# YihongSun/Dynamo-Depth

Measured on AMD Instinct MI355X. Metric: training images/sec (192x640 triplets), higher is better.
Workload: dtype f32

## Files before the change

### dynamo-depth_amd/hipops/abi.py

```python
import ctypes as C

DD_MAX_SCALES = 4
DD_NUM_SRC = 2
DD_ABI_VERSION = 2
DD_MODE_RIGID, DD_MODE_FLOW, DD_MODE_FLOW_MASK = 0, 1, 2
DD_PARTIAL_STRIDE = 40
DD_SUMS_STRIDE = 8

_fp = C.c_void_p


class DDPhotoScale(C.Structure):
    _fields_ = [
        ("shift", C.c_int), ("h", C.c_int), ("w", C.c_int),
        ("w_photo", C.c_float), ("w_cons", C.c_float),
        ("disp", _fp),
        ("flow", _fp * DD_NUM_SRC),
        ("mask", _fp * DD_NUM_SRC),
        ("noise", _fp),
        ("g_disp", _fp),
        ("g_flow", _fp * DD_NUM_SRC),
        ("g_mask", _fp * DD_NUM_SRC),
        ("out_color", _fp * DD_NUM_SRC),
        ("out_sample", _fp * DD_NUM_SRC),
# ... 123 lines not shown
        "dd_dwconv3x3_nhwc": (i, [v, v, i, i, i, i, i, v, v]),
        "dd_dwconv3x3_nhwc_bwd_data": (i, [v, v, i, i, i, i, i, v, v]),
        "dd_dwconv3x3_nhwc_bwd_weight": (i, [v, v, i, i, i, i, i, v, v, z, v]),
        "dd_dwconv3x3_workspace_bytes": (z, [i, i, i]),
        "dd_conv3x3_cout1_bwd_data": (i, [v, v, i, i, i, i, i, v, v]),
        "dd_prepare_frames": (i, [v, v, v, i, i, i, i, v, v, v, v]),
        "dd_prepare_frames_workspace_bytes": (z, [i, i]),
        "dd_pyramid_down2": (i, [v, i, i, i, v, v]),
        "dd_pack_rgb": (i, [v, i, i, i, v, v]),
        "dd_depth_metrics": (i, [v, i, i, i, v, v, i, v, C.POINTER(C.c_double), f, f, v, v, v, z, v]),
        "dd_depth_metrics_workspace_bytes": (z, [i, i]),
        "dd_depth_metrics_masked": (i, [v, i, i, i, v, v, i, v, C.POINTER(C.c_double), f, f, v, i, i, v, v, v, v, z, v]),
        "dd_depth_metrics_masked_workspace_bytes": (z, [i, i]),
        "dd_depth_metrics_accumulate": (i, [v, v, i, v, v, v]),
        "dd_odom_snippet_count": (i, [i, i]),
        "dd_odom_snippets": (i, [v, v, i, i, v, v, v]),
        "dd_motion_pr": (i, [v, i, i, i, v, v, i, i, v, i, i, v, v]),
        "dd_fill_contours": (i, [v, i, v, i, i, i, i, v, v]),
        "dd_vis_frame": (i, [v, v, v, v, v, v, v, v, f, f, i, i, C.POINTER(C.c_int), i, i, i, v, f, f, f, f, i, i, v, v, v, v]),
        "dd_vis_flow_tiles": (i, [v, v, C.POINTER(C.c_int), i, i, i, i, i, i, f, i, v, v]),
        "dd_bn_act_fwd": (i, [v, v, C.c_longlong, i, v, v, f, f, v, v, v, v, i, v, v, z, v]),
        "dd_bn_act_bwd": (i, [v, v, v, C.c_longlong, i, v, v, v, v, i, v, v, v, v, v, z, v]),
        "dd_bn_workspace_bytes": (z, [i]),
        "dd_bn_act_fwd_t": (i, [v, v, C.c_longlong, i, v, v, f, f, v, v, v, v, i, v, i, v, z, v]),
        "dd_bn_act_bwd_t": (i, [v, v, v, C.c_longlong, i, v, v, v, v, i, v, v, v, v, i, v, z, v]),
        "dd_channel_sum_nhwc_t": (i, [v, C.c_longlong, i, v, i, v, v]),
        "dd_reflect_pad1_nhwc_t": (i, [v, i, i, i, i, v, i, v]),
        "dd_reflect_pad1_nhwc_bwd_t": (i, [v, i, i, i, i, v, i, v]),
        "dd_up_cat_pad_t": (i, [v, v, i, i, i, i, i, i, i, v, i, v]),
        "dd_up_cat_pad_bwd_t": (i, [v, v, i, i, i, i, i, i, i, v, v, i, v]),
        "dd_layer_norm_fwd": (i, [v, C.c_longlong, i, v, v, f, v, v, v, v]),
        "dd_layer_norm_bwd": (i, [v, v, v, v, v, C.c_longlong, i, v, v, v, z, v]),
        "dd_layer_norm_workspace_bytes": (z, [i]),
        "dd_layer_scale_bwd": (i, [v, v, v, i, i, i, v, v, v, z, v]),
        "dd_layer_scale_workspace_bytes": (z, [i, i]),
        "dd_layer_norm_fwd_t": (i, [v, C.c_longlong, i, v, v, f, v, v, v, i, v]),
        "dd_layer_norm_bwd_t": (i, [v, v, v, v, v, C.c_longlong, i, v, v, v, z, i, v]),
        "dd_layer_scale_bwd_t": (i, [v, v, v, i, i, i, v, v, v, z, i, v]),
        "dd_layer_scale_fwd_t": (i, [v, v, v, i, i, i, v, i, v]),
        "dd_dwconv3x3_nhwc_t": (i, [v, v, i, i, i, i, i, v, i, v]),
        "dd_dwconv3x3_nhwc_bwd_data_t": (i, [v, v, i, i, i, i, i, v, i, v]),
        "dd_dwconv3x3_nhwc_bwd_weight_t": (i, [v, v, i, i, i, i, i, v, v, z, i, v]),
        "dd_redu_supported": (i, [i, i]),
        "dd_redu_workspace_bytes": (z, [C.c_longlong, i, i]),
        "dd_redu_fwd": (i, [v, v, v, v, C.c_longlong, i, i, v, v]),
        "dd_redu_bwd_data": (i, [v, v, C.c_longlong, i, i, v, v, v]),
        "dd_redu_bwd_weight": (i, [v, v, v, C.c_longlong, i, i, v, v, v, z, v]),
        "dd_conv_head_supported": (i, [i]),
        "dd_conv_head_workspace_bytes": (z, [i, i, i, i]),
        "dd_conv_head_fwd": (i, [v, v, C.c_longlong, C.c_longlong, C.c_longlong, v, i, i, i, i, v, v]),
        "dd_conv_head_bwd_weight": (i, [v, v, i, i, i, i, v, v, v, z, v]),
        "dd_conv_small_supported": (i, [i, i, i]),
        "dd_conv_small_workspace_bytes": (z, [i, i, i]),
        "dd_conv_small_fwd": (i, [v, v, C.c_longlong, C.c_longlong, C.c_longlong, C.c_longlong, v, i, i, i, i, i, i, v, v, z, v]),
        "dd_conv_small_bwd_data": (i, [v, v, C.c_longlong, C.c_longlong, C.c_longlong, C.c_longlong, i, i, i, i, i, i, v, v, z, v]),
        "dd_conv_small_bwd_weight": (i, [v, v, i, i, i, i, i, i, v, v, v, z, v]),
        "dd_conv3x3_mfma_supported": (i, [i, i]),
        "dd_conv3x3_mfma_pack_bytes": (z, [i, i]),
        "dd_conv3x3_mfma_pack": (i, [v, C.c_longlong, C.c_longlong, C.c_longlong, C.c_longlong, i, i, v, v, v]),
        "dd_conv3x3_mfma_pack_many_job_words": (i, []),
        "dd_conv3x3_mfma_pack_many_blocks": (i, [i, i, i, i]),
        "dd_conv3x3_mfma_pack_many": (i, [v, v, i, v]),
        "dd_conv3x3_mfma": (i, [v, v, v, i, i, i, i, i, i, v, v]),
        "dd_conv3x3_mfma_n": (i, [v, v, v, i, i, i, i, i, i, i, v, v]),
        "dd_conv3x3_mfma_flat_supported": (i, [i, i, i, i, i]),
        "dd_conv3x3_mfma_flat_workspace_bytes": (z, [i, i, i, i, i]),
        "dd_conv3x3_mfma_flat": (i, [v, v, v, i, i, i, i, i, v, v, z, v]),
        "dd_conv3x3_mfma_flat_n": (i, [v, v, v, i, i, i, i, i, i, v, v, z, v]),
        "dd_conv3x3_mfma_wgrad_workspace_bytes": (z, [i, i, i, i, i]),
        "dd_conv3x3_mfma_bwd_weight": (i, [v, v, i, i, i, i, i, i, v, v, z, v]),
        "dd_conv3x3_mfma_bwd_weight_n": (i, [v, v, i, i, i, i, i, i, i, v, v, z, v]),
        "dd_conv3x3_half_supported": (i, [i, i]),
        "dd_conv3x3_half_pack_bytes": (z, [i, i]),
        "dd_conv3x3_half_pack": (i, [v, C.c_longlong, C.c_longlong, C.c_longlong, C.c_longlong, i, i, i, v, v, v]),
        "dd_conv3x3_half": (i, [v, v, v, i, i, i, i, i, i, i, v, v]),
        "dd_conv3x3_half_wgrad_workspace_bytes": (z, [i, i, i, i, i]),
        "dd_conv3x3_half_bwd_weight": (i, [v, v, i, i, i, i, i, i, i, v, v, z, v]),
        "dd_pw_gemm_pack_bytes": (z, [i, i]),
        "dd_mlp_pack": (i, [v, C.c_longlong, C.c_longlong, v, C.c_longlong, C.c_longlong, i, i, v, v, v, v, v, v]),
        "dd_mlp_fwd_supported": (i, [i]),
        "dd_mlp_fwd": (i, [v, v, v, v, v, i, i, v, v]),
        "dd_pw_gemm": (i, [v, v, v, i, i, i, i, v, v]),
        "dd_gelu_pair": (i, [v, v, v, z, v]),
        "dd_adam_chunk": (i, []),
        "dd_adam_multi": (i, [v, i, v, i, v, C.c_double, C.c_double, C.c_double, C.c_double, C.c_double, v, v, v]),
        "dd_error_string": (C.c_char_p, [i]),
        "dd_abi_version": (i, []),
    }
    found = []
    for name, (res, args) in sig.items():
        try:
            fn = getattr(lib, name)
        except AttributeError:
            continue
        fn.restype = res
        fn.argtypes = args
        found.append(name)
    return found


EXPORTED = (
    "dd_photo_loss", "dd_photo_workspace_bytes", "dd_photo_timing", "dd_photo_timing_read", "dd_photo_loss_part", "dd_smooth_loss", "dd_smooth_workspace_bytes",
    "dd_ground_loss", "dd_ground_workspace_bytes", "dd_ground_plane", "dd_ground_candidates", "dd_ground_select",
    "dd_assemble_losses", "dd_reg_losses_finish", "dd_fused_loss", "dd_fused_loss_part", "dd_fused_loss_supported", "dd_reg_workspace_bytes", "dd_backproject", "dd_backproject_bwd", "dd_project3d", "dd_project3d_bwd", "dd_project3d_workspace_bytes",
    "dd_ssim", "dd_ssim_bwd", "dd_disp_to_depth", "dd_pose_matrix", "dd_pose_matrix_bwd",
    "dd_channel_sum_nhwc", "dd_channel_sum_workspace_bytes", "dd_reflect_pad1_nhwc", "dd_reflect_pad1_nhwc_bwd",
    "dd_dwconv3x3_nhwc", "dd_dwconv3x3_nhwc_bwd_data", "dd_dwconv3x3_nhwc_bwd_weight", "dd_dwconv3x3_workspace_bytes", "dd_conv3x3_cout1_bwd_data",
    "dd_prepare_frames", "dd_prepare_frames_workspace_bytes", "dd_pyramid_down2", "dd_pack_rgb", "dd_depth_metrics", "dd_depth_metrics_workspace_bytes", "dd_depth_metrics_masked", "dd_depth_metrics_masked_workspace_bytes", "dd_depth_metrics_accumulate", "dd_odom_snippet_count", "dd_odom_snippets", "dd_motion_pr", "dd_fill_contours", "dd_vis_frame", "dd_vis_flow_tiles", "dd_bn_act_fwd", "dd_bn_act_bwd", "dd_bn_workspace_bytes",
    "dd_bn_act_fwd_t", "dd_bn_act_bwd_t", "dd_channel_sum_nhwc_t", "dd_reflect_pad1_nhwc_t", "dd_reflect_pad1_nhwc_bwd_t", "dd_up_cat_pad_t", "dd_up_cat_pad_bwd_t",
    "dd_layer_norm_fwd", "dd_layer_norm_bwd", "dd_layer_norm_workspace_bytes", "dd_layer_scale_bwd", "dd_layer_scale_workspace_bytes",
    "dd_jpeg_workspace_bytes", "dd_jpeg_decode", "dd_resize_workspace_bytes", "dd_resize_bicubic", "dd_layer_norm_fwd_t", "dd_layer_norm_bwd_t", "dd_layer_scale_bwd_t", "dd_layer_scale_fwd_t", "dd_dwconv3x3_nhwc_t", "dd_dwconv3x3_nhwc_bwd_data_t",
    "dd_dwconv3x3_nhwc_bwd_weight_t", "dd_adam_chunk", "dd_adam_multi", "dd_conv_small_supported", "dd_conv_small_workspace_bytes",
    "dd_conv_small_fwd", "dd_conv_small_bwd_data", "dd_conv_small_bwd_weight", "dd_conv_head_supported", "dd_conv_head_workspace_bytes", "dd_conv_head_fwd",
    "dd_conv_head_bwd_weight", "dd_redu_supported", "dd_redu_workspace_bytes", "dd_redu_fwd", "dd_redu_bwd_data", "dd_redu_bwd_weight",
    "dd_conv3x3_mfma_supported", "dd_conv3x3_mfma_pack_bytes", "dd_conv3x3_mfma_pack", "dd_conv3x3_mfma_pack_many_job_words",
    "dd_conv3x3_mfma_pack_many_blocks", "dd_conv3x3_mfma_pack_many", "dd_conv3x3_mfma", "dd_conv3x3_mfma_n",
    "dd_conv3x3_mfma_flat_supported", "dd_conv3x3_mfma_flat_workspace_bytes", "dd_conv3x3_mfma_flat", "dd_conv3x3_mfma_flat_n",
    "dd_conv3x3_mfma_wgrad_workspace_bytes", "dd_conv3x3_mfma_bwd_weight", "dd_conv3x3_mfma_bwd_weight_n",
    "dd_conv3x3_half_supported", "dd_conv3x3_half_pack_bytes", "dd_conv3x3_half_pack", "dd_conv3x3_half",
    "dd_conv3x3_half_wgrad_workspace_bytes", "dd_conv3x3_half_bwd_weight",
    "dd_pw_gemm_pack_bytes", "dd_mlp_pack", "dd_pw_gemm", "dd_gelu_pair", "dd_mlp_fwd_supported", "dd_mlp_fwd",
    "dd_error_string", "dd_abi_version",
)


def fill_photo_args(*, B, H, W, mode, automask, want_grad, min_depth, max_depth, ssim_weight, eps, disp_thr,
                    target, source, K, inv_K, T, ts, g_T, sums, workspace, scales, source_packed=None):
    a = DDPhotoArgs()
    a.abi_version = DD_ABI_VERSION
    a.B, a.H, a.W = B, H, W
    a.num_scales = len(scales)
    a.mode, a.automask, a.want_grad = mode, int(bool(automask)), int(bool(want_grad))
    a.min_depth, a.max_depth, a.ssim_weight, a.eps, a.disp_thr = min_depth, max_depth, ssim_weight, eps, disp_thr
    a.target = ptr(target)
    a.K, a.inv_K = ptr(K), ptr(inv_K)
    a.sums, a.workspace = ptr(sums), ptr(workspace)
    for f in range(DD_NUM_SRC):
        a.source[f] = ptr(source[f])
        a.source_packed[f] = ptr(source_packed[f]) if source_packed is not None else None
        a.T[f] = ptr(T[f])
        a.ts[f] = ptr(ts[f]) if ts is not None else None
        a.g_T[f] = ptr(g_T[f]) if g_T is not None else None
    for s, d in enumerate(scales):
        sc = a.scale[s]
        sc.shift, sc.h, sc.w = d["shift"], d["h"], d["w"]
        sc.w_photo, sc.w_cons = d.get("w_photo", 0.0), d.get("w_cons", 0.0)
        for name in ("disp", "noise", "g_disp", "out_depth", "out_idsel"):
            setattr(sc, name, ptr(d.get(name)))
        for name in ("flow", "mask", "g_flow", "g_mask", "out_color", "out_sample", "out_resid", "out_delta"):
            pair = d.get(name) or (None, None)
            arr = getattr(sc, name)
            for f in range(DD_NUM_SRC):
                arr[f] = ptr(pair[f])
    return a
```

### dynamo-depth_amd/hipops/functions.py

```python
import os

import torch

from . import lib as L
from .pack_many import PackSet, _ACTIVE_PACK_SETS, _pack_many_on, pack_many_launches, pack_weights_once_per_forward


def _dev(t, name="tensor"):
    if not t.is_cuda:
        raise L.DynamoHipError("%s must live on the GPU: the Dynamo-Depth loss path has no CPU implementation "
                               "(libdynamo_hip.so is the only backend)" % name)
    if t.dtype != torch.float32:
        raise L.DynamoHipError("%s must be float32, got %s" % (name, t.dtype))
    return t.contiguous()


DTYPE_CODE = {torch.float32: 0, torch.float16: 1, torch.bfloat16: 2}


def _p(t):
    return None if t is None else t.data_ptr()


def _ws(nbytes, device):
    return torch.empty(max(int(nbytes) // 4, 1), dtype=torch.float32, device=device)


_WS_BYTES = {}


def _ws_bytes(name, *dims):
    key = (name,) + dims
    n = _WS_BYTES.get(key)
    if n is None:
        n = _WS_BYTES[key] = int(getattr(L.load(), name)(*dims))
    return n


def _nhwc_empty(B, Cc, H, W, device, *, dtype=torch.float32):
    return torch.empty((B, H, W, Cc), dtype=dtype, device=device).permute(0, 3, 1, 2)


def _channel_sum(g, rows, cout, code, stream):
    gb = torch.empty(cout, dtype=torch.float32, device=g.device)
    ws = _ws(_ws_bytes("dd_channel_sum_workspace_bytes", cout), g.device)
    L.check(L.load().dd_channel_sum_nhwc_t(_p(g), rows, cout, _p(gb), code, _p(ws), stream), "dd_channel_sum_nhwc_t")
    return gb


def _wgrad_1x1(go, x, w, B, H, W):
    cout, cin = w.shape
    _, gw, _ = torch.ops.aten.convolution_backward(go.view(B, H, W, cout).permute(0, 3, 1, 2), x.view(B, H, W, cin).permute(0, 3, 1, 2),
                                                   w.view(cout, cin, 1, 1), None, [1, 1], [0, 0], [1, 1], False, [0, 0], 1, [False, True, False])
    return gw.reshape(cout, cin)


def _wgrad_3x3_library(g, x, w_like, pad):
    return torch.ops.aten.convolution_backward(g, x, w_like, None, (1, 1), (pad, pad), (1, 1), False, [0, 0], 1, (False, True, False))[1]


def _conv3x3_s1(x, weight, stride, padding, dilation, groups, allowed):
    return (tuple(weight.shape[2:]) == (3, 3) and groups == 1 and tuple(stride) == (1, 1) and tuple(dilation) == (1, 1)
            and tuple(padding) in allowed and x.shape[1] == weight.shape[1])


def _below_tile_pixels(B, Ho, Wo, env_name):
    return Ho < 8 or Wo < 32 or B * Ho * Wo < int(os.environ.get(env_name, "20000"))


class BackprojectFn(torch.autograd.Function):

    @staticmethod
    def forward(ctx, depth, inv_K):
        depth, inv_K = _dev(depth, "depth"), _dev(inv_K, "inv_K")
        B, _, h, w = depth.shape
        pts = torch.empty(B, 4, h * w, dtype=torch.float32, device=depth.device)
        L.check(L.load().dd_backproject(_p(depth), _p(inv_K), B, h, w, _p(pts), L.current_stream()), "dd_backproject")
        ctx.save_for_backward(inv_K)
        ctx.shape = (B, h, w)
        return pts

    @staticmethod
    def backward(ctx, g):
        (inv_K,) = ctx.saved_tensors
        B, h, w = ctx.shape
        g = _dev(g, "grad")
        gd = torch.empty(B, 1, h, w, dtype=torch.float32, device=g.device)
        L.check(L.load().dd_backproject_bwd(_p(g), _p(inv_K), B, h, w, _p(gd), L.current_stream()), "dd_backproject_bwd")
        return gd, None


class Project3DFn(torch.autograd.Function):

    @staticmethod
    def forward(ctx, points, K, T, h, w, eps):
        points, K = _dev(points, "points"), _dev(K, "K")
        T = None if T is None else _dev(T, "T")
        B = points.shape[0]
        pix = torch.empty(B, h, w, 2, dtype=torch.float32, device=points.device)
        ego = torch.empty(B, 3, h * w, dtype=torch.float32, device=points.device)
        L.check(L.load().dd_project3d(_p(points), _p(K), _p(T), B, h, w, eps, _p(pix), _p(ego), L.current_stream()), "dd_project3d")
        ctx.save_for_backward(points, K, T if T is not None else torch.empty(0, device=points.device))
        ctx.has_T = T is not None
        ctx.dims = (B, h, w, eps)
        return pix, ego

    @staticmethod
    def backward(ctx, g_pix, g_ego):
        points, K, T = ctx.saved_tensors
        B, h, w, eps = ctx.dims
        T = T if ctx.has_T else None
        g_pix = None if g_pix is None else _dev(g_pix, "g_pix")
        g_ego = None if g_ego is None else _dev(g_ego, "g_ego")
        lib = L.load()
        g_points = torch.empty_like(points)
        g_T = torch.empty(B, 4, 4, dtype=torch.float32, device=points.device) if T is not None else None
        ws = _ws(lib.dd_project3d_workspace_bytes(B, h, w), points.device)
        L.check(lib.dd_project3d_bwd(_p(points), _p(K), _p(T), _p(g_pix), _p(g_ego), B, h, w, eps, _p(g_points), _p(g_T), _p(ws),
                                     L.current_stream()), "dd_project3d_bwd")
        return g_points, None, g_T, None, None, None


class SSIMFn(torch.autograd.Function):

    @staticmethod
    def forward(ctx, x, y):
        x, y = _dev(x, "x"), _dev(y, "y")
        B, Cc, H, W = x.shape
        out = torch.empty_like(x)
        L.check(L.load().dd_ssim(_p(x), _p(y), B, Cc, H, W, _p(out), L.current_stream()), "dd_ssim")
        ctx.save_for_backward(x, y)
        return out

    @staticmethod
    def backward(ctx, g):
        x, y = ctx.saved_tensors
        B, Cc, H, W = x.shape
# ... 562 lines not shown
    if os.environ.get("DD_STOCK_DECODER_GLUE", "0") == "1":
        return False
    if not (x.is_cuda and x.dtype in DTYPE_CODE and x.dim() == 4 and x.shape[1] % 4 == 0 and x.shape[1] >= 4 and _nhwc(x)
            and x.shape[2] >= 2 and x.shape[3] >= 2 and (mode != 2 or (x.shape[2] >= 4 and x.shape[3] >= 4))):
        return False
    if skip is not None:
        H, W = (x.shape[2], x.shape[3]) if mode == 2 else (2 * x.shape[2], 2 * x.shape[3])
        if not (skip.dtype == x.dtype and skip.is_cuda and skip.shape[0] == x.shape[0] and skip.shape[1] % 4 == 0 and tuple(skip.shape[2:]) == (H, W)
                and _nhwc(skip)):
            return False
    return True


def up_cat_pad(x, skip=None, mode="bilinear", elu=True):
    code = {"nearest": 0, "bilinear": 1, None: 2}[mode]
    if up_cat_pad_ok(x, skip, code):
        return UpCatPadFn.apply(x, skip, code, bool(elu))
    F = torch.nn.functional
    y = F.elu(x) if elu else x
    if mode is not None:
        y = F.interpolate(y, scale_factor=2, mode=mode)
    if skip is not None:
        y = torch.cat((y, skip), 1)
    return reflect_pad1(y)


class DepthwiseConv3x3NHWCFn(torch.autograd.Function):

    @staticmethod
    def forward(ctx, x, weight, dilation):
        B, Cc, H, W = x.shape
        w = weight.contiguous()
        out = torch.empty((B, Cc, H, W), dtype=x.dtype, device=x.device, memory_format=torch.channels_last)
        L.check(L.load().dd_dwconv3x3_nhwc_t(_p(x), _p(w), B, H, W, Cc, dilation, _p(out), DTYPE_CODE[x.dtype], L.current_stream()), "dd_dwconv3x3_nhwc_t")
        ctx.save_for_backward(x, w)
        ctx.dilation = dilation
        return out

    @staticmethod
    def backward(ctx, g):
        x, w = ctx.saved_tensors
        B, Cc, H, W = x.shape
        g = g.to(x.dtype).contiguous(memory_format=torch.channels_last)
        lib, gx, gw = L.load(), None, None
        code = DTYPE_CODE[x.dtype]
        if ctx.needs_input_grad[0]:
            gx = torch.empty((B, Cc, H, W), dtype=x.dtype, device=g.device, memory_format=torch.channels_last)
            L.check(lib.dd_dwconv3x3_nhwc_bwd_data_t(_p(g), _p(w), B, H, W, Cc, ctx.dilation, _p(gx), code, L.current_stream()), "dd_dwconv3x3_nhwc_bwd_data_t")
        if ctx.needs_input_grad[1]:
            gw = torch.empty_like(w)
            nbytes = _ws_bytes("dd_dwconv3x3_workspace_bytes", B, H, Cc)
            ws = _ws(nbytes, g.device)
            L.check(lib.dd_dwconv3x3_nhwc_bwd_weight_t(_p(g), _p(x), B, H, W, Cc, ctx.dilation, _p(gw), _p(ws), nbytes, code, L.current_stream()),
                    "dd_dwconv3x3_nhwc_bwd_weight_t")
        return gx, gw, None


def depthwise_conv3x3(x, weight, dilation):
    Cc = x.shape[1]
    if (x.is_cuda and x.dtype in DTYPE_CODE and weight.dtype == torch.float32 and x.dim() == 4 and Cc % 4 == 0 and Cc <= 512
            and x.is_contiguous(memory_format=torch.channels_last) and not x.is_contiguous()):
        return DepthwiseConv3x3NHWCFn.apply(x, weight, dilation)
    return torch.nn.functional.conv2d(x, weight, None, 1, dilation, dilation, Cc)


class PointwiseLinearFn(torch.autograd.Function):

    @staticmethod
    def forward(ctx, x, weight, bias):
        B, H, W, cin = x.shape
        ctx.save_for_backward(x, weight)
        with torch.autocast("cuda", enabled=False):
            return torch.addmm(bias, x.reshape(-1, cin), weight.t()).view(B, H, W, weight.shape[0])

    @staticmethod
    def backward(ctx, g):
        x, weight = ctx.saved_tensors
        B, H, W, cin = x.shape
        cout = weight.shape[0]
        g = g.to(x.dtype).contiguous()
        gx = gw = gb = None
        if ctx.needs_input_grad[0]:
            gx = torch.mm(g.view(-1, cout), weight).view(B, H, W, cin)
        if ctx.needs_input_grad[1]:
            gw = _wgrad_1x1(g, x, weight, B, H, W)
        if ctx.needs_input_grad[2]:
            gb = _channel_sum(g, B * H * W, cout, DTYPE_CODE[g.dtype], L.current_stream()).to(weight.dtype)
        return gx, gw, gb


def pointwise_linear(x, layer):
    if (x.is_cuda and x.dtype in DTYPE_CODE and layer.weight.dtype == torch.float32 and layer.bias is not None and x.dim() == 4
            and x.is_contiguous() and torch.is_grad_enabled() and layer.out_features <= 4096):
        if torch.is_autocast_enabled():
            dt = torch.get_autocast_dtype("cuda")
            return PointwiseLinearFn.apply(x.to(dt), layer.weight.to(dt), layer.bias.to(dt))
        if x.dtype == torch.float32:
            return PointwiseLinearFn.apply(x, layer.weight, layer.bias)
    return layer(x.reshape(-1, x.shape[-1])).view(*x.shape[:-1], layer.out_features)


_MLP_CALLS = [0]


def mlp_calls():
    return _MLP_CALLS[0]


def mlp_ok(y, block):
    if os.environ.get("DD_MLP", "0") != "1" or os.environ.get("DD_STOCK_MLP", "0") == "1" or torch.is_autocast_enabled():
        return False
    l1, l2 = block.pwconv1, block.pwconv2
    if y.dim() != 4 or y.shape[0] * y.shape[1] * y.shape[2] < int(os.environ.get("DD_MLP_MIN_ROWS", "16384")):
        return False
    return bool(y.is_cuda and y.dtype == torch.float32 and y.dim() == 4 and y.is_contiguous() and l1.weight.dtype == torch.float32
                and l1.bias is not None and l2.bias is not None and l1.in_features % 32 == 0 and l1.out_features % 32 == 0
                and l2.in_features == l1.out_features and l2.out_features == l1.in_features and y.shape[-1] == l1.in_features
                and isinstance(block.act, torch.nn.GELU) and getattr(block.act, "approximate", "none") == "none")


def _mlp_param_grads(needs, g, gpre, y, post, w1, w2, B, H, W, stream):
    M, code = B * H * W, DTYPE_CODE[torch.float32]
    gw1 = _wgrad_1x1(gpre, y, w1, B, H, W) if needs[1] else None
    gb1 = _channel_sum(gpre, M, w1.shape[0], code, stream) if needs[2] else None
    gw2 = _wgrad_1x1(g, post, w2, B, H, W) if needs[3] else None
    gb2 = _channel_sum(g, M, w2.shape[0], code, stream) if needs[4] else None
    return gw1, gb1, gw2, gb2


class MlpFn(torch.autograd.Function):

    @staticmethod
    def forward(ctx, y, w1, b1, w2, b2):
        lib = L.load()
        B, H, W, Cc = y.shape
        hid, M = w1.shape[0], B * H * W
        need = any(ctx.needs_input_grad)
        nb1, nb2 = _ws_bytes("dd_pw_gemm_pack_bytes", hid, Cc), _ws_bytes("dd_pw_gemm_pack_bytes", Cc, hid)
        packs = torch.empty(((nb1 + nb2) * (2 if need else 1)) // 4, dtype=torch.float32, device=y.device)
        p0 = packs.data_ptr()
        stream = L.current_stream()
        L.check(lib.dd_mlp_pack(_p(w1), w1.stride(0), w1.stride(1), _p(w2), w2.stride(0), w2.stride(1), Cc, hid, p0, p0 + nb1,
                                p0 + nb1 + nb2 if need else None, p0 + 2 * nb1 + nb2 if need else None, None, stream), "dd_mlp_pack")
        pre = torch.empty((M, hid), dtype=torch.float32, device=y.device)
        L.check(lib.dd_pw_gemm(_p(y), p0, _p(b1), M, Cc, hid, 0, _p(pre), stream), "dd_pw_gemm (pwconv1)")
        out = torch.empty((B, H, W, Cc), dtype=torch.float32, device=y.device)
        L.check(lib.dd_pw_gemm(_p(pre), p0 + nb1, _p(b2), M, hid, Cc, 1, _p(out), stream), "dd_pw_gemm (GELU, pwconv2)")
        _MLP_CALLS[0] += 1
        if need:
            ctx.save_for_backward(y, pre, w1, w2, packs)
        return out

    @staticmethod
    def backward(ctx, g):
        y, pre, w1, w2, packs = ctx.saved_tensors
        lib = L.load()
        B, H, W, Cc = y.shape
        hid, M = w1.shape[0], B * H * W
        nb1, nb2 = _ws_bytes("dd_pw_gemm_pack_bytes", hid, Cc), _ws_bytes("dd_pw_gemm_pack_bytes", Cc, hid)
        p0 = packs.data_ptr()
        stream = L.current_stream()
        g = g.to(torch.float32).contiguous()
        gpre = torch.empty((M, hid), dtype=torch.float32, device=g.device)
        L.check(lib.dd_pw_gemm(_p(g), p0 + nb1 + nb2, None, M, Cc, hid, 0, _p(gpre), stream), "dd_pw_gemm (g . w2)")
        post = torch.empty((M, hid), dtype=torch.float32, device=g.device)
        L.check(lib.dd_gelu_pair(_p(pre), _p(gpre), _p(post), M * hid, stream), "dd_gelu_pair")
        gy = None
        if ctx.needs_input_grad[0]:
            gy = torch.empty((B, H, W, Cc), dtype=torch.float32, device=g.device)
            L.check(lib.dd_pw_gemm(_p(gpre), p0 + 2 * nb1 + nb2, None, M, hid, Cc, 0, _p(gy), stream), "dd_pw_gemm (g_pre . w1)")
        return (gy,) + _mlp_param_grads(ctx.needs_input_grad, g, gpre, y, post, w1, w2, B, H, W, stream)


def mlp(y, block):
    return MlpFn.apply(y, block.pwconv1.weight, block.pwconv1.bias, block.pwconv2.weight, block.pwconv2.bias)


_MLP_FUSED_CALLS = [0]


def mlp_fused_calls():
    return _MLP_FUSED_CALLS[0]


def _mlp_block_ok(y, block):
    l1, l2 = block.pwconv1, block.pwconv2
    if not (y.is_cuda and y.dtype == torch.float32 and y.dim() == 4 and y.is_contiguous() and l1.weight.dtype == torch.float32):
        return False
    if y.shape[0] * y.shape[1] * y.shape[2] < int(os.environ.get("DD_MLP_FUSED_MIN_ROWS", "16384")):
        return False
    return bool(l1.bias is not None and l2.bias is not None and l1.out_features == 6 * l1.in_features and l2.in_features == l1.out_features
                and l2.out_features == l1.in_features and y.shape[-1] == l1.in_features and isinstance(block.act, torch.nn.GELU)
                and getattr(block.act, "approximate", "none") == "none" and L.load().dd_mlp_fwd_supported(l1.in_features))


def _mlp_fwd_launch(y, w1, b1, w2, b2):
    lib = L.load()
    B, H, W, Cc = y.shape
    hid, M = w1.shape[0], B * H * W
    nb1, nb2 = _ws_bytes("dd_pw_gemm_pack_bytes", hid, Cc), _ws_bytes("dd_pw_gemm_pack_bytes", Cc, hid)
    packs = torch.empty((nb1 + nb2) // 4, dtype=torch.float32, device=y.device)
    p0, stream = packs.data_ptr(), L.current_stream()
    L.check(lib.dd_mlp_pack(_p(w1), w1.stride(0), w1.stride(1), _p(w2), w2.stride(0), w2.stride(1), Cc, hid, p0, None, None, None, p0 + nb1, stream), "dd_mlp_pack")
    out = torch.empty((B, H, W, Cc), dtype=torch.float32, device=y.device)
    L.check(lib.dd_mlp_fwd(_p(y), p0, p0 + nb1, _p(b1), _p(b2), M, Cc, _p(out), stream), "dd_mlp_fwd")
    return out


def mlp_fused_ok(y, block):
# ... 239 lines not shown
```

### include/dynamo_hip.h

```cpp
#ifndef DYNAMO_HIP_H_
#define DYNAMO_HIP_H_

#include <stddef.h>
#include <stdint.h>

#ifdef __cplusplus
extern "C" {
#endif

#define DD_MAX_SCALES 4
#define DD_NUM_SRC 2
#define DD_ABI_VERSION 2

#define DD_MODE_RIGID 0
#define DD_MODE_FLOW 1
#define DD_MODE_FLOW_MASK 2

#define DD_PARTIAL_STRIDE 40
#define DD_SUMS_STRIDE 8

typedef struct DDPhotoScale {
  int shift;
  int h, w;
  float w_photo;
// ... 226 lines not shown
int dd_layer_norm_bwd(const float* x, const float* g_out, const float* gamma, const float* mean, const float* rstd, long long rows, int C,
                      float* g_x, float* g_gamma_beta, void* workspace, size_t workspace_bytes, void* stream);
size_t dd_layer_norm_workspace_bytes(int C);

int dd_layer_scale_bwd(const float* g_out, const float* y, const float* scale, int B, int rows, int C, float* g_y, float* g_scale,
                       void* workspace, size_t workspace_bytes, void* stream);
size_t dd_layer_scale_workspace_bytes(int B, int C);

int dd_layer_norm_fwd_t(const void* x, long long rows, int C, const float* gamma, const float* beta, float eps, void* y, float* mean, float* rstd,
                        int dtype, void* stream);
int dd_layer_norm_bwd_t(const void* x, const void* g_out, const float* gamma, const float* mean, const float* rstd, long long rows, int C,
                        void* g_x, float* g_gamma_beta, void* workspace, size_t workspace_bytes, int dtype, void* stream);
int dd_layer_scale_bwd_t(const void* g_out, const void* y, const float* scale, int B, int rows, int C, void* g_y, float* g_scale, void* workspace,
                         size_t workspace_bytes, int dtype, void* stream);
int dd_layer_scale_fwd_t(const void* res, const void* y, const float* scale, int B, int rows, int C, void* out, int dtype, void* stream);
int dd_dwconv3x3_nhwc_t(const void* x, const float* weight, int B, int H, int W, int C, int dilation, void* out, int dtype, void* stream);
int dd_dwconv3x3_nhwc_bwd_data_t(const void* g_out, const float* weight, int B, int H, int W, int C, int dilation, void* g_x, int dtype, void* stream);
int dd_dwconv3x3_nhwc_bwd_weight_t(const void* g_out, const void* x, int B, int H, int W, int C, int dilation, float* g_weight, void* workspace,
                                   size_t workspace_bytes, int dtype, void* stream);

int dd_redu_supported(int C, int cout);
size_t dd_redu_workspace_bytes(long long P, int C, int cout);
int dd_redu_fwd(const float* a, const float* b, const float* weight, const float* bias, long long P, int C, int cout, float* y, void* stream);
int dd_redu_bwd_data(const float* g_out, const float* weight, long long P, int C, int cout, float* g_a, float* g_b, void* stream);
int dd_redu_bwd_weight(const float* a, const float* b, const float* g_out, long long P, int C, int cout, float* g_weight, float* g_bias, void* workspace,
                       size_t workspace_bytes, void* stream);

int dd_conv_head_supported(int C);
size_t dd_conv_head_workspace_bytes(int B, int Hp, int Wp, int C);
int dd_conv_head_fwd(const float* x_padded, const float* weight, long long s_ci, long long s_kh, long long s_kw, const float* bias, int B, int Hp, int Wp,
                     int C, float* out, void* stream);
int dd_conv_head_bwd_weight(const float* x_padded, const float* g_out, int B, int Hp, int Wp, int C, float* g_weight, float* g_bias, void* workspace,
                            size_t workspace_bytes, void* stream);

int dd_conv_small_supported(int ks, int cin, int cout);
size_t dd_conv_small_workspace_bytes(int ks, int cin, int cout);
int dd_conv_small_fwd(const float* x, const float* weight, long long s_co, long long s_ci, long long s_kh, long long s_kw, const float* bias, int B, int H,
                      int W, int cin, int cout, int ks, float* y, void* workspace, size_t workspace_bytes, void* stream);
int dd_conv_small_bwd_data(const float* g_out, const float* weight, long long s_co, long long s_ci, long long s_kh, long long s_kw, int B, int H, int W, int cin,
                           int cout, int ks, float* g_x, void* workspace, size_t workspace_bytes, void* stream);
int dd_conv_small_bwd_weight(const float* x, const float* g_out, int B, int H, int W, int cin, int cout, int ks, float* g_weight, float* g_bias,
                             void* workspace, size_t workspace_bytes, void* stream);

int dd_conv3x3_mfma_supported(int cin, int cout);
size_t dd_conv3x3_mfma_pack_bytes(int n_out, int k_in);
int dd_conv3x3_mfma_pack(const float* weight, long long s_co, long long s_ci, long long s_kh, long long s_kw, int cout, int cin, void* pack_fwd,
                         void* pack_bwd_data, void* stream);
int dd_conv3x3_mfma_n(const float* x, const void* pack, const float* bias, int B, int Hi, int Wi, int k_in, int n_out, int pad, int products, float* y,
                      void* stream);
int dd_conv3x3_mfma_pack_many_job_words(void);
int dd_conv3x3_mfma_pack_many_blocks(int cout, int cin, int want_fwd, int want_bwd_data);
int dd_conv3x3_mfma_pack_many(const long long* jobs, const int* block_job, int n_blocks, void* stream);
int dd_conv3x3_mfma(const float* x, const void* pack, const float* bias, int B, int Hi, int Wi, int k_in, int n_out, int pad, float* y, void* stream);
int dd_conv3x3_mfma_flat_supported(int B, int H, int W, int k_in, int n_out);
size_t dd_conv3x3_mfma_flat_workspace_bytes(int B, int H, int W, int k_in, int n_out);
int dd_conv3x3_mfma_flat(const float* x, const void* pack, const float* bias, int B, int H, int W, int k_in, int n_out, float* y, void* workspace,
                         size_t workspace_bytes, void* stream);
int dd_conv3x3_mfma_flat_n(const float* x, const void* pack, const float* bias, int B, int H, int W, int k_in, int n_out, int products, float* y,
                           void* workspace, size_t workspace_bytes, void* stream);
size_t dd_conv3x3_mfma_wgrad_workspace_bytes(int B, int Ho, int Wo, int cin, int cout);
int dd_conv3x3_mfma_bwd_weight(const float* x, const float* g_out, int B, int Hi, int Wi, int cin, int cout, int pad, float* g_weight, void* workspace,
                               size_t workspace_bytes, void* stream);
int dd_conv3x3_mfma_bwd_weight_n(const float* x, const float* g_out, int B, int Hi, int Wi, int cin, int cout, int pad, int products, float* g_weight,
                                 void* workspace, size_t workspace_bytes, void* stream);

int dd_conv3x3_half_supported(int cin, int cout);
size_t dd_conv3x3_half_pack_bytes(int n_out, int k_in);
int dd_conv3x3_half_pack(const float* weight, long long s_co, long long s_ci, long long s_kh, long long s_kw, int cout, int cin, int dtype,
                         void* pack_fwd, void* pack_bwd_data, void* stream);
int dd_conv3x3_half(const void* x, const void* pack, const float* bias, int B, int Hi, int Wi, int k_in, int n_out, int pad, int dtype, void* y,
                    void* stream);
size_t dd_conv3x3_half_wgrad_workspace_bytes(int B, int Ho, int Wo, int cin, int cout);
int dd_conv3x3_half_bwd_weight(const void* x, const void* g_out, int B, int Hi, int Wi, int cin, int cout, int pad, int dtype, float* g_weight,
                               void* workspace, size_t workspace_bytes, void* stream);

size_t dd_pw_gemm_pack_bytes(int N, int K);
int dd_mlp_pack(const float* w1, long long s1_n, long long s1_k, const float* w2, long long s2_n, long long s2_k, int C, int hidden, void* pack_fwd1,
                void* pack_fwd2, void* pack_bwd2, void* pack_bwd1, void* pack_fwd2_fused, void* stream);
int dd_mlp_fwd_supported(int C);
int dd_mlp_fwd(const float* x, const void* pack_fwd1, const void* pack_fwd2_fused, const float* b1, const float* b2, int M, int C, float* y, void* stream);
int dd_pw_gemm(const float* x, const void* pack, const float* bias, int M, int K, int N, int gelu_in, float* y, void* stream);
int dd_gelu_pair(const float* pre, float* g_inout, float* post, size_t n, void* stream);

typedef struct DDAdamRecord {
  float* param;
  const float* grad;
  float* exp_avg;
  float* exp_avg_sq;
  float* step;
  long long n;
} DDAdamRecord;
int dd_adam_chunk(void);
int dd_adam_multi(const DDAdamRecord* records, int n_records, const int* block_map, int n_blocks, void* aux, double lr, double beta1, double beta2,
                  double eps, double weight_decay, const float* grad_scale, const float* found_inf, void* stream);

#define DD_VIS_MAX_TILES 16
#define DD_VIS_IMG 0
#define DD_VIS_REF_IMG 1
#define DD_VIS_DISP 2
#define DD_VIS_MASK 3
#define DD_VIS_EGO_FLOW 4
#define DD_VIS_IND_FLOW 5
#define DD_VIS_COMP_FLOW 6
#define DD_VIS_SAMP_FLOW 7
int dd_vis_frame(const float* color, const float* ref_color, const float* disp, const float* motion_mask, const float* complete_flow, const float* K,
                 const float* inv_K, const float* cam_T_cam, float min_depth, float max_depth, int H, int W, const int* tiles, int n_tiles, int R, int C,
                 const uint32_t* lut, float disp_vmin, float disp_vmax, float mask_vmin, float mask_vmax, int frame, int max_frames, uint8_t* panel,
                 float* side, float* maxima, void* stream);
int dd_vis_flow_tiles(const float* side, const float* maxima, const int* tiles, int n_tiles, int R, int C, int H, int W, int n_frames,
                      float flow_mag_factor, int consistent_flow, uint8_t* panel, void* stream);

const char* dd_error_string(int code);
int dd_abi_version(void);

#ifdef __cplusplus
}
#endif
#endif
```

Before: 362.0.

## Add split-K MFMA pointwise weight-gradient kernel fusing bias channel sums

Adds a custom HIP kernel that computes 1x1/linear weight gradients as a split-K GEMM over rows. It uses a 3-piece bf16 split of the fp32 inputs on MFMA 32x32x16 and double-buffered global prefetch. The bias channel sum is accumulated in the same pass, and a double-precision fold kernel reduces the partials. Linear and MLP backward route through it in place of the aten convolution_backward plus a separate channel-sum kernel, except for large-channel small-row shapes. This is meant to cut library overhead and an extra pass over the gradient, at the cost of a partial-sum workspace and an extra reduction launch.

```diff
diff --git a/dynamo-depth_amd/csrc/dd_pw_wgrad.hip b/dynamo-depth_amd/csrc/dd_pw_wgrad.hip
--- /dev/null
+++ b/dynamo-depth_amd/csrc/dd_pw_wgrad.hip
@@ -0,0 +1,308 @@
+#include <hip/hip_runtime.h>
+
+#include <cstdlib>
+#include <type_traits>
+
+#include "../../include/dynamo_hip.h"
+#include "dd_attr.h"
+#include "dd_split.h"
+
+namespace dd {
+namespace pwg {
+
+using cm::bf8;
+using cm::f16v;
+using cm::split2;
+
+constexpr int NT = 256;
+constexpr int KT = 32;
+constexpr int CSTR = KT * 2 + 16;
+
+template <int A, int B>
+constexpr int lds_bytes() { return 3 * 64 * (A + B) * CSTR; }
+
+template <int A, int B, int MINWG>
+__global__ __launch_bounds__(NT, MINWG) void pw_wgrad_kernel(const float* __restrict__ g, const float* __restrict__ x, int rows, int cout, int cin, int want_gb,
+                                                             float* __restrict__ partial) {
+  constexpr int TCO = 64 * A, TCI = 64 * B, G_PIECE = TCO * CSTR, X_PIECE = TCI * CSTR;
+  constexpr int GI = (A * B <= 3 || A < B) ? A : 1, GJ = (A * B <= 3 || A >= B) ? B : 1;
+  static_assert(lds_bytes<A, B>() >= A * 16 * 64 * 4, "the bias sums meet in the tile's LDS");
+  extern __shared__ __align__(16) unsigned char smem[];
+  unsigned char* const s_g = smem;
+  unsigned char* const s_x = smem + 3 * G_PIECE;
+  const int tid = threadIdx.x, lane = tid & 63, wave = __builtin_amdgcn_readfirstlane(tid >> 6);
+  const int wa = wave >> 1, wb = wave & 1;
+  const int ks = blockIdx.x, nks = gridDim.x, ci0 = blockIdx.y * TCI, co0 = blockIdx.z * TCO;
+  const int tiles = (rows + KT - 1) / KT;
+  const int t_begin = (int)((long long)tiles * ks / nks), t_end = (int)((long long)tiles * (ks + 1) / nks);
+
+  const int rp = ((tid >> 2) & 7) + 8 * ((tid >> 5) & 1), qc = (tid & 3) + 4 * (tid >> 6);
+  const int lds_off = (4 * qc) * CSTR + rp * 4;
+  bool g_ch[A], x_ch[B];
+#pragma unroll
+  for (int j = 0; j < A; ++j) g_ch[j] = __builtin_amdgcn_readfirstlane(co0 + 64 * j + 16 * wave) < cout;
+#pragma unroll
+  for (int j = 0; j < B; ++j) x_ch[j] = __builtin_amdgcn_readfirstlane(ci0 + 64 * j + 16 * wave) < cin;
+  const float* const g_src = g + co0 + 4 * qc;
+  const float* const x_src = x + ci0 + 4 * qc;
+
+  float4 pg[2][A][2], px[2][B][2];
+  const float4 zero4 = make_float4(0.f, 0.f, 0.f, 0.f);
+#pragma unroll
+  for (int j = 0; j < A; ++j) pg[0][j][0] = pg[0][j][1] = pg[1][j][0] = pg[1][j][1] = zero4;
+#pragma unroll
+  for (int j = 0; j < B; ++j) px[0][j][0] = px[0][j][1] = px[1][j][0] = px[1][j][1] = zero4;
+  bool row_ok[2][2] = {{false, false}, {false, false}};
+  auto keep = [](const float4& v, bool ok) { return make_float4(ok ? v.x : 0.f, ok ? v.y : 0.f, ok ? v.z : 0.f, ok ? v.w : 0.f); };
+  auto fetch = [&](int t, auto bufc) {
+    constexpr int b = decltype(bufc)::value;
+    const int r = t * KT + 2 * rp;
+    row_ok[b][0] = r < rows;
+    row_ok[b][1] = r + 1 < rows;
+    const size_t ra = (size_t)min(r, rows - 1), rb = (size_t)min(r + 1, rows - 1);
+#pragma unroll
+    for (int j = 0; j < A; ++j)
+      if (g_ch[j]) {
+        pg[b][j][0] = *reinterpret_cast<const float4*>(g_src + ra * cout + 64 * j);
+        pg[b][j][1] = *reinterpret_cast<const float4*>(g_src + rb * cout + 64 * j);
+      }
+#pragma unroll
+    for (int j = 0; j < B; ++j)
+      if (x_ch[j]) {
+        px[b][j][0] = *reinterpret_cast<const float4*>(x_src + ra * cin + 64 * j);
+        px[b][j][1] = *reinterpret_cast<const float4*>(x_src + rb * cin + 64 * j);
+      }
+  };
+  auto put = [&](unsigned char* plane, int piece_bytes, int off, const float4& a, const float4& b) {
+    const float av[4] = {a.x, a.y, a.z, a.w}, bv[4] = {b.x, b.y, b.z, b.w};
+#pragma unroll
+    for (int c = 0; c < 4; ++c) {
+      unsigned p1, p2, p3;
+      split2(av[c], bv[c], p1, p2, p3);
+      *reinterpret_cast<unsigned*>(plane + off + c * CSTR) = p1;
+      *reinterpret_cast<unsigned*>(plane + piece_bytes + off + c * CSTR) = p2;
+      *reinterpret_cast<unsigned*>(plane + 2 * piece_bytes + off + c * CSTR) = p3;
+    }
+  };
+  float4 bs[A];
+#pragma unroll
+  for (int j = 0; j < A; ++j) bs[j] = zero4;
+  auto stage = [&](auto bufc) {
+    constexpr int b = decltype(bufc)::value;
+#pragma unroll
+    for (int j = 0; j < A; ++j)
+      if (g_ch[j]) {
+        const float4 v0 = keep(pg[b][j][0], row_ok[b][0]), v1 = keep(pg[b][j][1], row_ok[b][1]);
+        bs[j].x += v0.x + v1.x;
+        bs[j].y += v0.y + v1.y;
+        bs[j].z += v0.z + v1.z;
+        bs[j].w += v0.w + v1.w;
+        put(s_g, G_PIECE, lds_off + 64 * j * CSTR, v0, v1);
+      }
+#pragma unroll
+    for (int j = 0; j < B; ++j)
+      if (x_ch[j]) put(s_x, X_PIECE, lds_off + 64 * j * CSTR, keep(px[b][j][0], row_ok[b][0]), keep(px[b][j][1], row_ok[b][1]));
+  };
+  auto lds_barrier = [&]() { asm volatile("s_waitcnt lgkmcnt(0)\n\ts_barrier" ::: "memory"); };
+
+  const int co_blocks = min((cout - co0) >> 5, 2 * A), ci_blocks = min((cin - ci0) >> 5, 2 * B);
+  const int na = __builtin_amdgcn_readfirstlane(max(0, (co_blocks - wa + 1) >> 1)), nb = __builtin_amdgcn_readfirstlane(max(0, (ci_blocks - wb + 1) >> 1));
+  f16v acc[A][B];
+#pragma unroll
+  for (int i = 0; i < A; ++i)
+#pragma unroll
+    for (int j = 0; j < B; ++j)
+#pragma unroll
+      for (int r = 0; r < 16; ++r) acc[i][j][r] = 0.f;
+
+  const unsigned char* a_lane = s_g + (wa * 32 + (lane & 31)) * CSTR + (lane >> 5) * 16;
+  const unsigned char* b_lane = s_x + (wb * 32 + (lane & 31)) * CSTR + (lane >> 5) * 16;
+
+  using Buf0 = std::integral_constant<int, 0>;
+  using Buf1 = std::integral_constant<int, 1>;
+  auto tile = [&](int t, auto bufc) {
+    lds_barrier();
+    stage(bufc);
+    lds_barrier();
+    if (t + 2 < t_end) fetch(t + 2, bufc);
+#pragma unroll
+    for (int s = 0; s < 2; ++s) {
+#pragma unroll
+      for (int i0 = 0; i0 < A; i0 += GI)
+#pragma unroll
+        for (int j0 = 0; j0 < B; j0 += GJ) {
+          uint4 af[GI][3], bf[GJ][3];
+#pragma unroll
+          for (int gi = 0; gi < GI; ++gi)
+#pragma unroll
+            for (int pc = 0; pc < 3; ++pc) af[gi][pc] = *reinterpret_cast<const uint4*>(a_lane + (i0 + gi) * 64 * CSTR + s * 32 + pc * G_PIECE);
+#pragma unroll
+          for (int gj = 0; gj < GJ; ++gj)
+#pragma unroll
+            for (int pc = 0; pc < 3; ++pc) bf[gj][pc] = *reinterpret_cast<const uint4*>(b_lane + (j0 + gj) * 64 * CSTR + s * 32 + pc * X_PIECE);
+          f16v tmp[GI][GJ];
+#pragma unroll
+          for (int gi = 0; gi < GI; ++gi)
+#pragma unroll
+            for (int gj = 0; gj < GJ; ++gj)
+#pragma unroll
+              for (int r = 0; r < 16; ++r) tmp[gi][gj][r] = 0.f;
+#pragma unroll
+          for (int tt = 0; tt < 6; ++tt)
+#pragma unroll
+            for (int gi = 0; gi < GI; ++gi)
+#pragma unroll
+              for (int gj = 0; gj < GJ; ++gj)
+                if (i0 + gi < na && j0 + gj < nb)
+                  tmp[gi][gj] = __builtin_amdgcn_mfma_f32_32x32x16_bf16(__builtin_bit_cast(bf8, af[gi][cm::kPieceA[tt]]),
+                                                                        __builtin_bit_cast(bf8, bf[gj][cm::kPieceB[tt]]), tmp[gi][gj], 0, 0, 0);
+#pragma unroll
+          for (int gi = 0; gi < GI; ++gi)
+#pragma unroll
+            for (int gj = 0; gj < GJ; ++gj)
+              if (i0 + gi < na && j0 + gj < nb) {
+#pragma unroll
+                for (int r = 0; r < 16; ++r) acc[i0 + gi][j0 + gj][r] += tmp[gi][gj][r];
+              }
+          if (GI * GJ < A * B) __builtin_amdgcn_sched_barrier(0);
+        }
+    }
+  };
+  if (t_begin < t_end) fetch(t_begin, Buf0{});
+  if (t_begin + 1 < t_end) fetch(t_begin + 1, Buf1{});
+  for (int t = t_begin; t < t_end; t += 2) {
+    tile(t, Buf0{});
+    if (t + 1 < t_end) tile(t + 1, Buf1{});
+  }
+
+  float* const P = partial + (size_t)ks * ((size_t)cout * cin + cout);
+#pragma unroll
+  for (int i = 0; i < A; ++i)
+#pragma unroll
+    for (int j = 0; j < B; ++j)
+      if (i < na && j < nb) {
+        float* dst = P + (size_t)(co0 + (2 * i + wa) * 32 + 4 * (lane >> 5)) * cin + ci0 + (2 * j + wb) * 32 + (lane & 31);
+#pragma unroll
+        for (int r = 0; r < 16; ++r) dst[(size_t)((r & 3) + 8 * (r >> 2)) * cin] = acc[i][j][r];
+      }
+
+  if (want_gb && blockIdx.y == 0) {
+    float* const red = reinterpret_cast<float*>(smem);
+    lds_barrier();
+#pragma unroll
+    for (int j = 0; j < A; ++j) *reinterpret_cast<float4*>(red + (j * 16 + rp) * 64 + 4 * qc) = bs[j];
+    lds_barrier();
+    for (int c = tid; c < TCO; c += NT) {
+      const float* col = red + (c >> 6) * 16 * 64 + (c & 63);
+      float s = 0.f;
+#pragma unroll
+      for (int k = 0; k < 16; ++k) s += col[k * 64];
+      if (co0 + c < cout) P[(size_t)cout * cin + co0 + c] = s;
+    }
+  }
+}
+
+constexpr int FOLD_W = 16;
+__global__ __launch_bounds__(FOLD_W * 64) void pw_wgrad_fold_kernel(const float* __restrict__ partial, int nks, int n_w, int n_all, size_t pstride,
+                                                                    float* __restrict__ gw, float* __restrict__ gb) {
+  __shared__ double red[FOLD_W][64];
+  const int lane = threadIdx.x & 63, wave = threadIdx.x >> 6;
+  const int idx = blockIdx.x * 64 + lane;
+  const bool in = idx < n_all;
+  double s[4] = {0., 0., 0., 0.};
+  if (in) {
+    const float* P = partial + idx;
+    int k = wave;
+    for (; k + 3 * FOLD_W < nks; k += 4 * FOLD_W) {
+#pragma unroll
+      for (int j = 0; j < 4; ++j) s[j] += (double)P[(size_t)(k + FOLD_W * j) * pstride];
+    }
+    for (; k < nks; k += FOLD_W) s[0] += (double)P[(size_t)k * pstride];
+  }
+  red[wave][lane] = (s[0] + s[1]) + (s[2] + s[3]);
+  __syncthreads();
+  if (wave == 0 && in) {
+    double v = 0.;
+#pragma unroll
+    for (int w = 0; w < FOLD_W; w += 4) v += (red[w][lane] + red[w + 1][lane]) + (red[w + 2][lane] + red[w + 3][lane]);
+    if (idx < n_w) gw[idx] = (float)v;
+    else gb[idx - n_w] = (float)v;
+  }
+}
+
+struct Tile {
+  int a, b;
+};
+
+static Tile tile_for(int cout, int cin) {
+  if (const char* e = std::getenv("DD_PW_WGRAD_TILE")) {
+    switch (std::atoi(e)) {
+      case 0: return {2, 2};
+      case 1: return {3, 1};
+      case 2: return {1, 3};
+    }
+  }
+  if (cout <= 128 && cin <= 128) return {2, 2};
+  return cout >= cin ? Tile{3, 1} : Tile{1, 3};
+}
+
+static int splits_for(int rows, int cout, int cin) {
+  const Tile t = tile_for(cout, cin);
+  const int groups = ((cout + 64 * t.a - 1) / (64 * t.a)) * ((cin + 64 * t.b - 1) / (64 * t.b));
+  const int tiles = (rows + KT - 1) / KT;
+  int n = 512 / groups;
+  if (const char* e = std::getenv("DD_PW_WGRAD_SPLITS")) n = std::atoi(e);
+  const int min_tiles = tiles >= 64 ? 4 : 1;
+  if (n > tiles / min_tiles) n = tiles / min_tiles;
+  return n < 1 ? 1 : n;
+}
+
+template <int A, int B>
+static int launch(const float* g, const float* x, int rows, int cout, int cin, int want_gb, int nks, float* partial, hipStream_t s) {
+  auto kern = pw_wgrad_kernel<A, B, 2>;
+  constexpr int lds = lds_bytes<A, B>();
+  static dd::LdsAttrOnce lds_attr;
+  if (const int rc = lds_attr.ensure(reinterpret_cast<const void*>(kern), lds)) return rc;
+  const dim3 grid(nks, (cin + 64 * B - 1) / (64 * B), (cout + 64 * A - 1) / (64 * A));
+  hipLaunchKernelGGL(kern, grid, dim3(NT), lds, s, g, x, rows, cout, cin, want_gb, partial);
+  return (int)hipGetLastError();
+}
+
+}
+}
+
+extern "C" int dd_pw_wgrad_supported(int cout, int cin) {
+  return (cout >= 32 && cin >= 32 && cout % 32 == 0 && cin % 32 == 0 && cout <= 4096 && cin <= 4096) ? 1 : 0;
+}
+
+extern "C" size_t dd_pw_wgrad_workspace_bytes(int rows, int cout, int cin) {
+  if (rows < 1 || !dd_pw_wgrad_supported(cout, cin)) return 0;
+  return (size_t)dd::pwg::splits_for(rows, cout, cin) * ((size_t)cout * cin + cout) * sizeof(float);
+}
+
+extern "C" int dd_pw_wgrad_n(const float* g, const float* x, int rows, int cout, int cin, int products, float* gw, float* gb, void* workspace,
+                             size_t workspace_bytes, void* stream) {
+  using namespace dd::pwg;
+  if (!g || !x || !gw || !workspace || rows < 1 || !dd_pw_wgrad_supported(cout, cin) || products != 6) return (int)hipErrorInvalidValue;
+  if (workspace_bytes < dd_pw_wgrad_workspace_bytes(rows, cout, cin)) return (int)hipErrorInvalidValue;
+  if ((reinterpret_cast<unsigned long long>(g) | reinterpret_cast<unsigned long long>(x) | reinterpret_cast<unsigned long long>(workspace)) & 15ull)
+    return (int)hipErrorInvalidValue;
+  hipStream_t s = static_cast<hipStream_t>(stream);
+  const Tile t = tile_for(cout, cin);
+  const int nks = splits_for(rows, cout, cin), want_gb = gb ? 1 : 0;
+  float* part = static_cast<float*>(workspace);
+  int rc;
+  if (t.a == 2) rc = launch<2, 2>(g, x, rows, cout, cin, want_gb, nks, part, s);
+  else if (t.a == 3) rc = launch<3, 1>(g, x, rows, cout, cin, want_gb, nks, part, s);
+  else rc = launch<1, 3>(g, x, rows, cout, cin, want_gb, nks, part, s);
+  if (rc != 0) return rc;
+  const int n_w = cout * cin, n_all = n_w + (want_gb ? cout : 0);
+  hipLaunchKernelGGL(pw_wgrad_fold_kernel, dim3((n_all + 63) / 64), dim3(FOLD_W * 64), 0, s, static_cast<const float*>(workspace), nks, n_w, n_all,
+                     (size_t)cout * cin + cout, gw, gb);
+  return (int)hipGetLastError();
+}
+
+extern "C" int dd_pw_wgrad(const float* g, const float* x, int rows, int cout, int cin, float* gw, float* gb, void* workspace, size_t workspace_bytes,
+                           void* stream) {
+  return dd_pw_wgrad_n(g, x, rows, cout, cin, 6, gw, gb, workspace, workspace_bytes, stream);
+}
diff --git a/dynamo-depth_amd/hipops/abi.py b/dynamo-depth_amd/hipops/abi.py
--- a/dynamo-depth_amd/hipops/abi.py
+++ b/dynamo-depth_amd/hipops/abi.py
@@ -229,6 +229,10 @@
         "dd_mlp_fwd": (i, [v, v, v, v, v, i, i, v, v]),
         "dd_pw_gemm": (i, [v, v, v, i, i, i, i, v, v]),
         "dd_gelu_pair": (i, [v, v, v, z, v]),
+        "dd_pw_wgrad_supported": (i, [i, i]),
+        "dd_pw_wgrad_workspace_bytes": (z, [i, i, i]),
+        "dd_pw_wgrad": (i, [v, v, i, i, i, v, v, v, z, v]),
+        "dd_pw_wgrad_n": (i, [v, v, i, i, i, i, v, v, v, z, v]),
         "dd_adam_chunk": (i, []),
         "dd_adam_multi": (i, [v, i, v, i, v, C.c_double, C.c_double, C.c_double, C.c_double, C.c_double, v, v, v]),
         "dd_error_string": (C.c_char_p, [i]),
@@ -267,6 +271,7 @@
     "dd_conv3x3_half_supported", "dd_conv3x3_half_pack_bytes", "dd_conv3x3_half_pack", "dd_conv3x3_half",
     "dd_conv3x3_half_wgrad_workspace_bytes", "dd_conv3x3_half_bwd_weight",
     "dd_pw_gemm_pack_bytes", "dd_mlp_pack", "dd_pw_gemm", "dd_gelu_pair", "dd_mlp_fwd_supported", "dd_mlp_fwd",
+    "dd_pw_wgrad_supported", "dd_pw_wgrad_workspace_bytes", "dd_pw_wgrad", "dd_pw_wgrad_n",
     "dd_error_string", "dd_abi_version",
 )
 
diff --git a/dynamo-depth_amd/hipops/functions.py b/dynamo-depth_amd/hipops/functions.py
--- a/dynamo-depth_amd/hipops/functions.py
+++ b/dynamo-depth_amd/hipops/functions.py
@@ -53,6 +53,35 @@
     _, gw, _ = torch.ops.aten.convolution_backward(go.view(B, H, W, cout).permute(0, 3, 1, 2), x.view(B, H, W, cin).permute(0, 3, 1, 2),
                                                    w.view(cout, cin, 1, 1), None, [1, 1], [0, 0], [1, 1], False, [0, 0], 1, [False, True, False])
     return gw.reshape(cout, cin)
+
+
+_PW_WGRAD_CALLS = [0]
+
+
+def pw_wgrad_calls():
+    return _PW_WGRAD_CALLS[0]
+
+
+def _pw_wgrad_library_wins(rows, cout, cin):
+    return rows < 16384 and cout * cin > 65536
+
+
+def _linear_param_grads(g, x, w, need_w, need_b):
+    B, H, W, cout = g.shape
+    cin, rows = x.shape[-1], B * H * W
+    if (need_w and g.dtype == torch.float32 and x.dtype == torch.float32 and w.dtype == torch.float32 and not torch.is_autocast_enabled()
+            and os.environ.get("DD_STOCK_PW_WGRAD", "0") != "1"
+            and rows < (1 << 31) and not _pw_wgrad_library_wins(rows, cout, cin) and mfma_products() == 6 and L.load().dd_pw_wgrad_supported(cout, cin)):
+        gw = torch.empty((cout, cin), dtype=torch.float32, device=g.device)
+        gb = torch.empty(cout, dtype=torch.float32, device=g.device) if need_b else None
+        nbytes = _ws_bytes("dd_pw_wgrad_workspace_bytes", rows, cout, cin)
+        ws = _ws(nbytes, g.device)
+        L.check(L.load().dd_pw_wgrad(_p(g), _p(x), rows, cout, cin, _p(gw), _p(gb), _p(ws), nbytes, L.current_stream()), "dd_pw_wgrad")
+        _PW_WGRAD_CALLS[0] += 1
+        return gw, gb
+    gw = _wgrad_1x1(g, x, w, B, H, W) if need_w else None
+    gb = _channel_sum(g, rows, cout, DTYPE_CODE[g.dtype], L.current_stream()).to(w.dtype) if need_b else None
+    return gw, gb
 
 
 def _wgrad_3x3_library(g, x, w_like, pad):
@@ -781,10 +810,7 @@
         gx = gw = gb = None
         if ctx.needs_input_grad[0]:
             gx = torch.mm(g.view(-1, cout), weight).view(B, H, W, cin)
-        if ctx.needs_input_grad[1]:
-            gw = _wgrad_1x1(g, x, weight, B, H, W)
-        if ctx.needs_input_grad[2]:
-            gb = _channel_sum(g, B * H * W, cout, DTYPE_CODE[g.dtype], L.current_stream()).to(weight.dtype)
+        gw, gb = _linear_param_grads(g, x, weight, ctx.needs_input_grad[1], ctx.needs_input_grad[2])
         return gx, gw, gb
 
 
@@ -819,11 +845,9 @@
 
 
 def _mlp_param_grads(needs, g, gpre, y, post, w1, w2, B, H, W, stream):
-    M, code = B * H * W, DTYPE_CODE[torch.float32]
-    gw1 = _wgrad_1x1(gpre, y, w1, B, H, W) if needs[1] else None
-    gb1 = _channel_sum(gpre, M, w1.shape[0], code, stream) if needs[2] else None
-    gw2 = _wgrad_1x1(g, post, w2, B, H, W) if needs[3] else None
-    gb2 = _channel_sum(g, M, w2.shape[0], code, stream) if needs[4] else None
+    hid = w1.shape[0]
+    gw1, gb1 = _linear_param_grads(gpre.view(B, H, W, hid), y.view(B, H, W, -1), w1, needs[1], needs[2])
+    gw2, gb2 = _linear_param_grads(g.view(B, H, W, -1), post.view(B, H, W, hid), w2, needs[3], needs[4])
     return gw1, gb1, gw2, gb2
 
 
diff --git a/include/dynamo_hip.h b/include/dynamo_hip.h
--- a/include/dynamo_hip.h
+++ b/include/dynamo_hip.h
@@ -332,6 +332,12 @@
 int dd_pw_gemm(const float* x, const void* pack, const float* bias, int M, int K, int N, int gelu_in, float* y, void* stream);
 int dd_gelu_pair(const float* pre, float* g_inout, float* post, size_t n, void* stream);
 
+int dd_pw_wgrad_supported(int cout, int cin);
+size_t dd_pw_wgrad_workspace_bytes(int rows, int cout, int cin);
+int dd_pw_wgrad(const float* g, const float* x, int rows, int cout, int cin, float* gw, float* gb, void* workspace, size_t workspace_bytes, void* stream);
+int dd_pw_wgrad_n(const float* g, const float* x, int rows, int cout, int cin, int products, float* gw, float* gb, void* workspace,
+                  size_t workspace_bytes, void* stream);
+
 typedef struct DDAdamRecord {
   float* param;
   const float* grad;
```

After: 365.5 (median of 6 runs). About the same (+1.0%).
